# Meng-333/SRADSGAN

Measured on AMD Instinct MI355X. Metric: training images/sec (216x216, x4), higher is better.
Workload: dtype f32 (split-bf16 products: 3 bf16 MFMA terms per fp32 multiply, fp32 accumulate)

## Files before the change

### sradsgan_amd/csrc/conv_api.hip

```cpp
#include "conv_internal.h"
#include "conv_dev.h"

using namespace srhip;

namespace srhip {
struct PackEntry {
  const float* w;
  float* packed;
  int cout, cin, kh, kw, mode, fast;
};
__global__ __launch_bounds__(256) void pack_batched_kernel(const PackEntry* __restrict__ tab) {
  const PackEntry e = tab[blockIdx.y];
  const int khkw = e.kh * e.kw;
  if (e.fast) {
    constexpr int LDS_F = 32 * (16 * 9 + 1);
    __shared__ float tile[LDS_F];
    const long total = (long)e.cout * e.cin * khkw;
    const int RO = e.mode == 0 ? 8 : 32;
    const int CI = e.mode == 0 ? (khkw <= 9 ? 64 : 16) : (khkw <= 9 ? 16 : 4);
    const int ld = CI * khkw + 1;
    const int nci = (e.cin + CI - 1) / CI, nco = (e.cout + RO - 1) / RO;
    const int ndst = e.mode == 0 ? e.cout : e.cin, csrc = e.mode == 0 ? e.cin : e.cout;
    const long ndst16 = ((long)ndst + 15) / 16 * 16;
    float* s0 = e.packed;
    char* s1 = reinterpret_cast<char*>(e.packed + total);
    char* s2 = reinterpret_cast<char*>(e.packed + 2 * total);
    char* s3 = reinterpret_cast<char*>(e.packed + 3 * total);
    for (int t = blockIdx.x; t < nci * nco; t += gridDim.x) {
      const int co0 = (t / nci) * RO, ci0 = (t % nci) * CI;
      const int cw = min(CI, e.cin - ci0), rw = min(RO, e.cout - co0);
      const int rowlen = cw * khkw;
      __syncthreads();
      for (int i = threadIdx.x; i < rw * rowlen; i += 256) {
        const int r = i / rowlen, k = i - r * rowlen;
        tile[r * ld + k] = e.w[((size_t)(co0 + r) * e.cin + ci0) * khkw + k];
      }
      __syncthreads();
      auto at = [&](int a, int b, int tap) { return tile[a * ld + b * khkw + tap]; };
      const int nn = e.mode == 0 ? rw : cw, nc = e.mode == 0 ? cw : rw;
      const int n0 = e.mode == 0 ? co0 : ci0, c00 = e.mode == 0 ? ci0 : co0;
      for (int it = threadIdx.x; it < nn * khkw * (nc / 8); it += 256) {
        const int g8 = it % (nc / 8), rt = it / (nc / 8);
        const int tap = rt % khkw, dn = rt / khkw;
        float v[8];
#pragma unroll
        for (int j = 0; j < 8; ++j) v[j] = e.mode == 0 ? at(dn, g8 * 8 + j, tap) : at(g8 * 8 + j, dn, tap);
        const long idx = ((long)(n0 + dn) * khkw + tap) * csrc + c00 + g8 * 8;
        reinterpret_cast<float4*>(s0 + idx)[0] = make_float4(v[0], v[1], v[2], v[3]);
        reinterpret_cast<float4*>(s0 + idx)[1] = make_float4(v[4], v[5], v[6], v[7]);
        bf16x8_t hi, lo;
        split_bf16x8(make_float4(v[0], v[1], v[2], v[3]), make_float4(v[4], v[5], v[6], v[7]), hi, lo);
        *reinterpret_cast<u32x4*>(s1 + idx * 4) = __builtin_bit_cast(u32x4, hi);
        *reinterpret_cast<u32x4*>(s1 + idx * 4 + 16) = __builtin_bit_cast(u32x4, lo);
        const f16x8_t f16 = {(_Float16)v[0], (_Float16)v[1], (_Float16)v[2], (_Float16)v[3], (_Float16)v[4], (_Float16)v[5], (_Float16)v[6], (_Float16)v[7]};
        const u32x4 z = {0u, 0u, 0u, 0u};
        *reinterpret_cast<u32x4*>(s2 + idx * 4) = __builtin_bit_cast(u32x4, f16);
        *reinterpret_cast<u32x4*>(s2 + idx * 4 + 16) = z;
      }
      for (int it = threadIdx.x; it < nn * khkw * (nc / 16); it += 256) {
        const int dn = it % nn, rt = it / nn;
        const int tap = rt % khkw, g16 = rt / khkw;
        const int n = n0 + dn, swz = (n >> 2) & 3;
        char* row = s3 + (((long)((c00 >> 4) + g16) * khkw + tap) * ndst16 + n) * 64;
#pragma unroll
        for (int h = 0; h < 2; ++h) {
          float v[8];
#pragma unroll
          for (int j = 0; j < 8; ++j) v[j] = e.mode == 0 ? at(dn, g16 * 16 + h * 8 + j, tap) : at(g16 * 16 + h * 8 + j, dn, tap);
          bf16x8_t hi, lo;
          split_bf16x8(make_float4(v[0], v[1], v[2], v[3]), make_float4(v[4], v[5], v[6], v[7]), hi, lo);
          *reinterpret_cast<u32x4*>(row + (((2 * h) ^ swz) << 4)) = __builtin_bit_cast(u32x4, hi);
          *reinterpret_cast<u32x4*>(row + (((2 * h + 1) ^ swz) << 4)) = __builtin_bit_cast(u32x4, lo);
        }
      }
    }
  } else {
    const int csrc = e.mode == 0 ? e.cin : e.cout, cdst = e.mode == 0 ? e.cout : e.cin;
    const int ld = ((cdst + 31) / 32) * 32;
    const long total = (long)khkw * csrc * ld;
    for (long idx = (long)blockIdx.x * blockDim.x + threadIdx.x; idx < total; idx += (long)gridDim.x * blockDim.x) {
      const int row = (int)(idx / ld), col = (int)(idx - (long)row * ld);
      float v = 0.f;
      if (col < cdst) {
        const int tap = row / csrc, cs = row - tap * csrc;
        const int a = tap / e.kw, b = tap - a * e.kw;
        if (e.mode == 0)
          v = e.w[(((size_t)col * e.cin + cs) * e.kh + a) * e.kw + b];
        else
          v = e.w[(((size_t)cs * e.cin + col) * e.kh + (e.kh - 1 - a)) * e.kw + (e.kw - 1 - b)];
      }
      e.packed[idx] = v;
    }
  }
}
}

namespace srhip {
extern int g_fast_cfg;
extern int g_wgrad_cfg;
extern int g_rowtap_addr;
extern int g_rowtap_pipe;
extern int g_patch_ks;
extern int g_fast_dynlds;
extern int g_fast_ablate;
extern int g_conv_math;
extern int g_sgam_cfg;
extern int g_pers_grid;
extern int g_pers_small;
extern int g_pool_epi_any;
extern int g_pers_abl;
extern int g_phase_batch;
extern int g_headconv_rows;
}
extern int g_tail_dbg;
namespace srhip {
}

namespace srhip {
struct Probe {
  int kind = 0, n = 0, h = 0, w = 0, cin = 0, cout = 0, cap = 0, count = 0;
  hipEvent_t ev[2 * 1024];
  int units[1024];
  int created = 0;
};
static Probe g_probe;
static inline bool probe_hit(int kind, int n, int h, int w, int cin, int cout) {
  return g_probe.kind == kind && g_probe.count < g_probe.cap && g_probe.n == n && g_probe.h == h && g_probe.w == w && g_probe.cin == cin &&
         g_probe.cout == cout;
}
static inline int probe_begin(void* stream) {
  const int i = g_probe.count;
  (void)hipEventRecord(g_probe.ev[2 * i], as_stream(stream));
  return i;
}
static inline void probe_end(int i, void* stream, int units = 1) {
  (void)hipEventRecord(g_probe.ev[2 * i + 1], as_stream(stream));
  g_probe.units[i] = units;
  g_probe.count = i + 1;
}
}

extern "C" {

int srhip_probe_config(int kind, int n, int h, int w, int cin, int cout, int max_pairs) {
  SRHIP_REQUIRE(kind >= 0 && kind <= 3 && max_pairs >= 0 && max_pairs <= 1024, "probe_config: kind 0..3, max_pairs <= 1024");
  while (g_probe.created < 2 * max_pairs) {
    if (hipEventCreate(&g_probe.ev[g_probe.created]) != hipSuccess) {
      set_error("probe_config: hipEventCreate failed");
      return SRHIP_ERR_LAUNCH;
    }
    ++g_probe.created;
  }
  g_probe.kind = kind; g_probe.n = n; g_probe.h = h; g_probe.w = w; g_probe.cin = cin; g_probe.cout = cout;
  g_probe.cap = kind ? max_pairs : 0;
  g_probe.count = 0;
  return SRHIP_OK;
}
int srhip_probe_read(float* ms, int* units, int cap) {
  SRHIP_REQUIRE(ms || cap == 0, "probe_read: null buffer");
  const int n = g_probe.count < cap ? g_probe.count : cap;
  for (int i = 0; i < n; ++i) {
    if (hipEventSynchronize(g_probe.ev[2 * i + 1]) != hipSuccess || hipEventElapsedTime(&ms[i], g_probe.ev[2 * i], g_probe.ev[2 * i + 1]) != hipSuccess) {
      set_error("probe_read: event %d not readable", i);
      return -1;
    }
    if (units) units[i] = g_probe.units[i];
  }
  return n;
}

int srhip_debug_set(int key, int value) {
  if (key == 0) {
    g_fast_cfg = value;
    return SRHIP_OK;
  }
  if (key == 1) {
    g_wgrad_cfg = value;
    return SRHIP_OK;
  }
  if (key == 2) {
    g_fast_dynlds = value;
    return SRHIP_OK;
  }
  if (key == 3) {
    g_fast_ablate = value;
    return SRHIP_OK;
  }
  if (key == 4) {
    g_sgam_cfg = value;
    return SRHIP_OK;
  }
  if (key == 5) {
    g_pers_grid = value;
    return SRHIP_OK;
  }
  if (key == 6) {
    g_pers_abl = value;
    return SRHIP_OK;
  }
  if (key == 7) {
    g_tail_dbg = value;
    return SRHIP_OK;
  }
  if (key == 8) {
    g_rowtap_addr = value;
    return SRHIP_OK;
  }
  if (key == 9) {
    g_rowtap_pipe = value;
    return SRHIP_OK;
  }
  if (key == 10) {
    g_patch_ks = value;
    return SRHIP_OK;
  }
  if (key == 11) {
    g_pers_small = value;
    return SRHIP_OK;
  }
  if (key == 12) {
    g_flat_blocks = value > 0 ? value : 768;
    return SRHIP_OK;
  }
  if (key == 13) {
    g_flat_abl = value;
    return SRHIP_OK;
  }
  if (key == 14) {
    g_flat_f32_k8 = value;
    return SRHIP_OK;
  }
  if (key == 15) {
    g_patch8 = value;
    return SRHIP_OK;
  }
  if (key == 16) {
    g_patch8_abl = value;
    return SRHIP_OK;
  }
  if (key == 17) {
    g_phase_batch = value;
    return SRHIP_OK;
  }
  if (key == 18) {
    g_headconv_rows = value;
    return SRHIP_OK;
  }
  if (key == 19) {
    g_pool_epi_any = value;
    return SRHIP_OK;
  }
  return SRHIP_ERR_ARG;
}

int srhip_set_conv_math(int mode) {
  SRHIP_REQUIRE(mode == SRHIP_MATH_FP32 || mode == SRHIP_MATH_BF16X3 || mode == SRHIP_MATH_HALF, "set_conv_math: unknown mode");
  g_conv_math = mode;
  return SRHIP_OK;
}
int srhip_get_conv_math(void) { return g_conv_math; }

size_t srhip_packed_elems(int cout, int cin, int kh, int kw, int mode) {
  if (cout <= 0 || cin <= 0 || kh <= 0 || kw <= 0 || (mode != 0 && mode != 1)) return 0;
  const bool fast = mode == 0 ? fast_fwd_ok(cin, cout, kh, kw) : fast_dgrad_ok(cin, cout, kh, kw);
  if (fast)
    return 3 * (size_t)cout * cin * kh * kw + (size_t)fast_tiled_elems(mode == 0 ? cout : cin, mode == 0 ? cin : cout, kh * kw);
  const int csrc = mode == 0 ? cin : cout, cdst = mode == 0 ? cout : cin;
  return (size_t)kh * kw * csrc * legacy_packed_ld(cdst);
}

int srhip_pack_entry_bytes(void) { return (int)sizeof(PackEntry); }

int srhip_packed_is_fast(int cout, int cin, int kh, int kw, int mode) {
  return (mode == 0 ? fast_fwd_ok(cin, cout, kh, kw) : fast_dgrad_ok(cin, cout, kh, kw)) ? 1 : 0;
}

int srhip_pack_weights_batched(const void* entries_dev, int count, void* stream) {
  SRHIP_REQUIRE(entries_dev && count >= 0, "pack_weights_batched: bad argument");
  if (count == 0) return SRHIP_OK;
  hipLaunchKernelGGL(pack_batched_kernel, dim3(32, count), dim3(256), 0, as_stream(stream),
                     static_cast<const PackEntry*>(entries_dev));
  return check_launch("pack_weights_batched");
}

int srhip_pack_weight(const float* w, float* packed, int cout, int cin, int kh, int kw, int mode, void* stream) {
  SRHIP_REQUIRE(w && packed && cout > 0 && cin > 0 && kh > 0 && kw > 0 && (mode == 0 || mode == 1),
                "pack_weight: bad argument");
  const bool fast = mode == 0 ? fast_fwd_ok(cin, cout, kh, kw) : fast_dgrad_ok(cin, cout, kh, kw);
  if (fast) return fast_pack_weight(w, packed, cout, cin, kh, kw, mode, as_stream(stream));
  return legacy_pack_weight(w, packed, cout, cin, kh, kw, mode, stream);
}

int srhip_conv2d_fwd(const float* x, const float* packed, const float* bias, const float* residual,
                     const float* rowscale, const float* chanscale, float* y, int n, int h, int w, int cin, int cout, int kh, int kw,
                     int stride, int pad, int ldx, int ldy, int ldr, float slope, int flags, void* stream) {
  SRHIP_REQUIRE(x && packed && y, "conv2d_fwd: null tensor");
  SRHIP_REQUIRE(n >= 0 && h > 0 && w > 0 && cin > 0 && cout > 0 && kh > 0 && kw > 0 && stride > 0 && pad >= 0,
                "conv2d_fwd: bad geometry");
  SRHIP_REQUIRE(ldx >= cin && ldy >= cout, "conv2d_fwd: row stride smaller than channel count");
  SRHIP_REQUIRE(!(flags & SRHIP_EPI_BIAS) || bias, "conv2d_fwd: EPI_BIAS without bias");
  SRHIP_REQUIRE(!(flags & SRHIP_EPI_RESIDUAL) || (residual && ldr >= cout), "conv2d_fwd: EPI_RESIDUAL without residual");
  SRHIP_REQUIRE(!(flags & SRHIP_EPI_ROWSCALE) || rowscale, "conv2d_fwd: EPI_ROWSCALE without rowscale");
  SRHIP_REQUIRE(!(flags & SRHIP_EPI_CHANSCALE) || chanscale, "conv2d_fwd: EPI_CHANSCALE without chanscale");
  if (fast_fwd_ok(cin, cout, kh, kw)) {
    const bool pr = probe_hit(1, n, h, w, cin, cout);
    const int pi = pr ? probe_begin(stream) : 0;
    const int rc = fast_conv2d_fwd(x, packed, bias, residual, rowscale, chanscale, y, n, h, w, cin, cout, kh, kw, stride, pad, ldx, ldy,
                                   ldr, slope, flags, as_stream(stream));
    if (pr) probe_end(pi, stream);
    return rc;
  }
  SRHIP_REQUIRE(!(flags & SRHIP_EPI_CHANSCALE), "conv2d_fwd: EPI_CHANSCALE needs Cin % 16 == 0");
  return legacy_conv2d_fwd(x, packed, bias, residual, rowscale, y, n, h, w, cin, cout, kh, kw, stride, pad, ldx, ldy,
                           ldr, slope, flags, stream);
}

int srhip_conv2d_fwd_dual(const float* x, const float* packed, const float* bias, const float* residual, const float* rowscale,
                          const float* chanscale, float* y, void* y_pp, int* served, int n, int h, int w, int cin, int cout, int kh,
                          int kw, int stride, int pad, int ldx, int ldy, int ldr, float slope, int flags, void* stream) {
  SRHIP_REQUIRE(y_pp && served && (((uintptr_t)y_pp) & 15) == 0 && ldy == cout, "conv2d_fwd_dual: 16-byte aligned plane buffer, dense fp32 output");
  g_dst2_req.pp = y_pp;
  g_dst2_req.served = 0;
  const int rc = srhip_conv2d_fwd(x, packed, bias, residual, rowscale, chanscale, y, n, h, w, cin, cout, kh, kw, stride, pad, ldx, ldy, ldr,
                                  slope, flags, stream);
  *served = g_dst2_req.served;
  g_dst2_req.pp = nullptr;
  g_dst2_req.served = 0;
  return rc;
}

int srhip_conv2d_fwd_pool(const float* x, const float* packed, const float* bias, float* y, float* pool, size_t pool_sec_bytes,
                          int* nseg_out, int n, int h, int w, int cin, int cout, int ldx, int ldy, int flags, void* stream) {
  SRHIP_REQUIRE(x && packed && y && pool && nseg_out, "conv2d_fwd_pool: null tensor");
  SRHIP_REQUIRE(cout == 64 && ldy == 64 && n > 0 && h > 0 && w > 0 && cin > 0 && ldx >= cin, "conv2d_fwd_pool: 64 dense destination channels");
  SRHIP_REQUIRE((flags & ~SRHIP_EPI_BIAS) == 0 && (!(flags & SRHIP_EPI_BIAS) || bias), "conv2d_fwd_pool: plain or bias epilogue");
  SRHIP_REQUIRE(pool_sec_bytes % 16 == 0 && pool_sec_bytes < (1u << 30) && (((uintptr_t)pool) & 15) == 0 &&
                    pool_sec_bytes >= (size_t)n * POOL_MAXSEG * 64 * sizeof(float),
                "conv2d_fwd_pool: three 16-byte aligned sections of n * max_segments * 64 floats");
  g_pool_req.out = pool;
  g_pool_req.sec_bytes = (unsigned)pool_sec_bytes;
  g_pool_req.served_nseg = 0;
  const int rc = srhip_conv2d_fwd(x, packed, bias, nullptr, nullptr, nullptr, y, n, h, w, cin, cout, 3, 3, 1, 1, ldx, ldy, 0, 0.f, flags, stream);
  const int served = g_pool_req.served_nseg;
  g_pool_req.out = nullptr;
  g_pool_req.served_nseg = 0;
  if (rc != SRHIP_OK) return rc;
  if (served > 0) {
    *nseg_out = served;
    return SRHIP_OK;
  }
  *nseg_out = srhip_clam_pool_segments();
  return srhip_clam_pool_partial(y, pool, pool_sec_bytes, n, h, w, cout, stream);
}

int srhip_conv2d_dgrad(const float* dy, const float* packed, float* dx, const float* residual, const float* actmask,
                       float slope, int n, int h, int w, int cin, int cout, int kh, int kw, int stride, int pad,
                       int ldy, int ldx, int ldr, int accumulate, void* stream) {
  SRHIP_REQUIRE(dy && packed && dx, "conv2d_dgrad: null tensor");
  SRHIP_REQUIRE(n >= 0 && h > 0 && w > 0 && cin > 0 && cout > 0 && kh > 0 && kw > 0 && stride > 0 && pad >= 0,
                "conv2d_dgrad: bad geometry");
  SRHIP_REQUIRE(pad <= kh - 1 && pad <= kw - 1, "conv2d_dgrad: pad > kernel-1 unsupported");
  SRHIP_REQUIRE(ldy >= cout && ldx >= cin, "conv2d_dgrad: row stride smaller than channel count");
  SRHIP_REQUIRE(!residual || ldr >= cin, "conv2d_dgrad: residual row stride smaller than channel count");
  if (fast_dgrad_ok(cin, cout, kh, kw)) {
    const bool pr = probe_hit(2, n, h, w, cin, cout);
    const int pi = pr ? probe_begin(stream) : 0;
    const int rc = fast_conv2d_dgrad(dy, packed, dx, residual, actmask, slope, n, h, w, cin, cout, kh, kw, stride, pad, ldy,
                                     ldx, ldr, accumulate, as_stream(stream));
    if (pr) probe_end(pi, stream);
    return rc;
  }
  SRHIP_REQUIRE(!residual && !actmask, "conv2d_dgrad: fused residual/activation mask needs Cout % 16 == 0");
  return legacy_conv2d_dgrad(dy, packed, dx, n, h, w, cin, cout, kh, kw, stride, pad, ldy, ldx, accumulate, stream);
}

static int add_unserved_residuals(float* dx, const float* r2, const float* r3, long count, void* stream) {
  const float* tab[3] = {dx, r2 ? r2 : r3, r3};
  const int k = 1 + (r2 ? 1 : 0) + (r3 ? 1 : 0);
  if (k == 1) return SRHIP_OK;
  return srhip_sum_n(tab, k, dx, count, stream);
}
int srhip_conv2d_dgrad_res3(const float* dy, const float* packed, float* dx, const float* residual, const float* residual2,
                            const float* residual3, int n, int h, int w, int cin, int cout, int kh, int kw, int stride, int pad,
                            void* stream) {
  SRHIP_REQUIRE(residual && (residual2 || residual3), "conv2d_dgrad_res3: residual and at least one more");
  SRHIP_REQUIRE(cin % 4 == 0 && ((((uintptr_t)residual2) | ((uintptr_t)residual3) | ((uintptr_t)dx)) & 15) == 0, "conv2d_dgrad_res3: Cin % 4 == 0, 16-byte aligned tensors");
  g_res_req.r2 = residual2 ? residual2 : residual3;
  g_res_req.r3 = residual2 ? residual3 : nullptr;
  g_res_req.served = 0;
  const int rc = srhip_conv2d_dgrad(dy, packed, dx, residual, nullptr, 0.f, n, h, w, cin, cout, kh, kw, stride, pad, cout, cin, cin, 0, stream);
  const bool served = g_res_req.served != 0;
  g_res_req = ResRequest();
  if (rc != SRHIP_OK || served) return rc;
  return add_unserved_residuals(dx, residual2, residual3, (long)n * h * w * cin, stream);
}
int srhip_conv2d_dgrad_pp_res3(const void* dy, int dy_pp, const float* packed, float* dx, const float* residual, const float* residual2,
                               const float* residual3, int n, int h, int w, int cin, int cout, void* stream) {
  SRHIP_REQUIRE(residual && (residual2 || residual3), "conv2d_dgrad_pp_res3: residual and at least one more");
  SRHIP_REQUIRE(cin % 4 == 0 && ((((uintptr_t)residual2) | ((uintptr_t)residual3)) & 15) == 0, "conv2d_dgrad_pp_res3: Cin % 4 == 0, 16-byte aligned tensors");
  g_res_req.r2 = residual2 ? residual2 : residual3;
  g_res_req.r3 = residual2 ? residual3 : nullptr;
  g_res_req.served = 0;
// ... 209 lines not shown
```

### sradsgan_amd/csrc/conv_fast.hip

```cpp
#include "conv_dev.h"

namespace srhip {

int g_fast_ablate = 0;



template <int BM, int BN, int WM, int WN, int BK, int MATH = 0>
__global__ __launch_bounds__(WM* WN * 64) void fast_conv_kernel(const float* __restrict__ src,
                                                                 const float* __restrict__ wt,
                                                                 const float* __restrict__ bias,
                                                                 const float* __restrict__ residual,
                                                                 const float* __restrict__ rowscale,
                                                                 const float* __restrict__ chanscale,
                                                                 const float* __restrict__ actmask,
                                                                 float* __restrict__ dst, FastGeom g, int nblk_m,
                                                                 int nblk_n) {
  constexpr int NT = WM * WN * 64;
  constexpr int WTM = BM / WM, WTN = BN / WN;
  constexpr int TM = WTM / 32, TN = WTN / 32;
  constexpr int LS = BK + 4;
  constexpr int QPR = BK / 4;
  constexpr int RPP = NT / QPR;
  constexpr int AR = (BM + RPP - 1) / RPP, BR = (BN + RPP - 1) / RPP;
// ... 443 lines not shown
#pragma unroll
  for (int t = 0; t < TM; ++t) {
    const int m = m0 + wm * WTM + t * 32 + l31;
    csrow[t] = chanscale + (size_t)((m < g.M ? m : 0) / OHOW) * g.C + khalf * 4;
  }
  const int T_taps = g.TH * g.TW;
  int c_tap = 0, c_cc = 0;

  auto chunk_sync = [&](int kc) {
    if (kc + 1 < nk)
      asm volatile("s_waitcnt vmcnt(%0)" ::"n"(AI + BI) : "memory");
    else
      asm volatile("s_waitcnt vmcnt(0)" ::: "memory");
    __builtin_amdgcn_s_barrier();
    asm volatile("" ::: "memory");
  };
  auto read_frags = [&](int stage, float4 (&af)[2][TM], float4 (&bf)[2][TN]) {
    const char* sb = lds + stage * STAGE_B;
#pragma unroll
    for (int t = 0; t < TM; ++t) af[0][t] = *reinterpret_cast<const float4*>(sb + aoff[t]);
#pragma unroll
    for (int u = 0; u < TN; ++u) bf[0][u] = *reinterpret_cast<const float4*>(sb + boff[u]);
#pragma unroll
    for (int t = 0; t < TM; ++t) af[1][t] = *reinterpret_cast<const float4*>(sb + (aoff[t] ^ (MATH ? 16 : 32)));
#pragma unroll
    for (int u = 0; u < TN; ++u) bf[1][u] = *reinterpret_cast<const float4*>(sb + (boff[u] ^ (MATH ? 16 : 32)));
    if (cscale) {
#pragma unroll
      for (int ks = 0; ks < 2; ++ks)
#pragma unroll
        for (int t = 0; t < TM; ++t) {
          const float4 sc = *reinterpret_cast<const float4*>(csrow[t] + c_cc * BK + (MATH ? ks * 4 + khalf * 4 : ks * 8));
          af[ks][t].x *= sc.x;
          af[ks][t].y *= sc.y;
          af[ks][t].z *= sc.z;
          af[ks][t].w *= sc.w;
        }
      if (++c_tap == T_taps) {
        c_tap = 0;
        ++c_cc;
      }
    }
  };

  if (MATH == 0 && nk > 0) {
    issue(0);
    if (nk > 1) issue(1);
    int stage = 0, nstage = 2;
    for (int kc = 0; kc < nk; ++kc) {
      chunk_sync(kc);
      if (kc + 2 < nk) issue(nstage);
      float4 af[2][TM], bf[2][TN];
      read_frags(stage, af, bf);
#pragma unroll
      for (int ks = 0; ks < 2; ++ks) {
#pragma unroll
        for (int t = 0; t < TM; ++t)
#pragma unroll
          for (int u = 0; u < TN; ++u) acc[t][u] = mfma32f(af[ks][t].x, bf[ks][u].x, acc[t][u]);
#pragma unroll
        for (int t = 0; t < TM; ++t)
#pragma unroll
          for (int u = 0; u < TN; ++u) acc[t][u] = mfma32f(af[ks][t].y, bf[ks][u].y, acc[t][u]);
#pragma unroll
        for (int t = 0; t < TM; ++t)
#pragma unroll
          for (int u = 0; u < TN; ++u) acc[t][u] = mfma32f(af[ks][t].z, bf[ks][u].z, acc[t][u]);
#pragma unroll
        for (int t = 0; t < TM; ++t)
#pragma unroll
          for (int u = 0; u < TN; ++u) acc[t][u] = mfma32f(af[ks][t].w, bf[ks][u].w, acc[t][u]);
      }
      stage = stage == 2 ? 0 : stage + 1;
      nstage = nstage == 2 ? 0 : nstage + 1;
    }
  }
  if (MATH >= 1 && nk > 0) {
    constexpr int PROD = MATH >= 1 ? MATH - 1 : 0;
    issue(0);
    if (nk > 1) issue(1);
    int stage = 0, nstage = 2;
    for (int kc = 0; kc < nk; ++kc) {
      chunk_sync(kc);
      if (kc + 2 < nk) issue(nstage);
      float4 af[2][TM], bf[2][TN];
      read_frags(stage, af, bf);
      bf16x8_t ah[TM], al[TM], bh[TN], bl[TN];
#pragma unroll
      for (int t = 0; t < TM; ++t) {
        if (PROD == 0) split_bf16x8(af[0][t], af[1][t], ah[t], al[t]);
        else ah[t] = al[t] = round16x8<PROD>(af[0][t], af[1][t]);
      }
#pragma unroll
      for (int u = 0; u < TN; ++u) {
        bh[u] = __builtin_bit_cast(bf16x8_t, bf[0][u]);
        bl[u] = PROD == 0 ? __builtin_bit_cast(bf16x8_t, bf[1][u]) : bh[u];
      }
#pragma unroll
      for (int i = 0; i < nprod<PROD>() * TM * TN; ++i) {
        const int grp = PROD == 0 ? i / (TM * TN) : 2, t = (i % (TM * TN)) / TN, u = i % TN;
        acc[t][u] = mma16<PROD>(grp == 0 ? al[t] : ah[t], grp == 1 ? bl[u] : bh[u], acc[t][u]);
      }
      stage = stage == 2 ? 0 : stage + 1;
      nstage = nstage == 2 ? 0 : nstage + 1;
    }
  }

  const int flags = EPI >= 0 ? EPI : g.flags;
  __syncthreads();
  float* wl = reinterpret_cast<float*>(lds) + wave * (32 * WTN);
  constexpr int QPRW = WTN / 4;
  constexpr int NRD = 32 * QPRW / 64;
#pragma unroll
  for (int t = 0; t < TM; ++t) {
#pragma unroll
    for (int u = 0; u < TN; ++u)
#pragma unroll
      for (int r = 0; r < 16; ++r) wl[((r & 3) + 8 * (r >> 2) + 4 * khalf) * WTN + u * 32 + l31] = acc[t][u][r];
    asm volatile("s_waitcnt lgkmcnt(0)" ::: "memory");
    constexpr int EB = NRD < 4 ? NRD : 4;
#pragma unroll
    for (int i0 = 0; i0 < NRD; i0 += EB) {
      float4 vq[EB];
      EpiOps eo[EB];
      unsigned dpx[EB];
      int nq[EB];
      bool okq[EB];
#pragma unroll
      for (int j = 0; j < EB; ++j) {
        const int idx = (i0 + j) * 64 + lane;
        const int row = idx / QPRW, cq = idx - row * QPRW;
        vq[j] = *reinterpret_cast<const float4*>(wl + row * WTN + cq * 4);
        const int m = m0 + wm * WTM + t * 32 + row;
        nq[j] = n0 + wn * WTN + cq * 4;
        okq[j] = m < g.M && nq[j] < g.K;
        size_t dpix = (size_t)(okq[j] ? m : 0);
        if (!g.dst_identity) {
          const int mm = okq[j] ? m : 0;
          const int nimg = mm / OHOW;
          const int rem = mm - nimg * OHOW;
          const int oh = rem / g.OW;
          const int ow = rem - oh * g.OW;
          dpix = ((size_t)nimg * g.Hd + (oh * g.dsd + g.ph)) * g.Wd + (ow * g.dsd + g.pw);
        }
        dpx[j] = (unsigned)dpix;
        if (!okq[j]) nq[j] = 0;
        eo[j] = epi_fetch(dpix, nq[j], flags, g, bias, residual, rowscale, actmask, dst, EPI < 0 && g.accumulate != 0);
      }
#pragma unroll
      for (int j = 0; j < EB; ++j)
        if (okq[j]) epi_finish(vq[j], eo[j], dpx[j], nq[j], flags, g, dst, EPI < 0 && g.accumulate != 0);
    }
    if (t + 1 < TM) asm volatile("s_waitcnt lgkmcnt(0)" ::: "memory");
  }
}


template <int BN, int EPI, int PROD = 0>
__global__ __launch_bounds__(256) __attribute__((amdgpu_waves_per_eu(3))) void conv_patch_kernel(const float* __restrict__ src, const float* __restrict__ wt,
                                                          const float* __restrict__ bias,
                                                          const float* __restrict__ residual,
                                                          const float* __restrict__ actmask, float* __restrict__ dst,
                                                          FastGeom g, PatchGeom pg, int nblk_m, int nblk_n) {
  constexpr int NW = 4, BK = 16;
  constexpr int WTM = 64, WTN = BN / 2;
  constexpr int TM = WTM / 32, TN = WTN / 32;
  constexpr int BPW = BN / 64;
  constexpr int MAXP = 3;
  constexpr int PATCH_B = 12 * 1024;
  constexpr int BSTAGE_B = BN * 64;
  constexpr int EPI_B = NW * 32 * WTN * 4;
  constexpr int LDS_B = 2 * PATCH_B + 3 * BSTAGE_B > EPI_B ? 2 * PATCH_B + 3 * BSTAGE_B : EPI_B;
  __shared__ __attribute__((aligned(1024))) char lds[LDS_B];
  __shared__ int pix_tab[128];

  const int tid = threadIdx.x, lane = tid & 63;
  const int wave = __builtin_amdgcn_readfirstlane(tid >> 6);
  const int tile = xcd_tile(blockIdx.x, nblk_m * nblk_n);
  const int tile_n = tile % nblk_n, pid = tile / nblk_n;
  const int n0 = tile_n * BN;
  const int tpi = pg.tiles_h * pg.tiles_w;
  const int img = pid / tpi;
  const int prem = pid - img * tpi;
  const int ty = prem / pg.tiles_w, tx = prem - ty * pg.tiles_w;
  const int oh0 = ty * pg.PH, ow0 = tx * pg.PW;
  const unsigned lds_base = (unsigned)(size_t)(__attribute__((address_space(3))) char*)lds;
  if (tid < 128) {
    int pr_, pc_;
    patch_pixel(tid, pg.PH, pg.PW, pg.gmap, pr_, pc_);
    pix_tab[tid] = (pr_ << 16) | pc_;
  }
  __syncthreads();

  const int swz = (lane >> 4) & 3;
  const int aq = (lane & 3) ^ swz;
  int abase[MAXP];
#pragma unroll
  for (int k = 0; k < MAXP; ++k) {
    const int row = (k * NW + wave) * 16 + (lane >> 2);
    abase[k] = -1;
    if (row < pg.PR) {
      const int pi = row / pg.PWP, pj = row - pi * pg.PWP;
      const int sh = oh0 + pg.lo_h + pi, sw = ow0 + pg.lo_w + pj;
      if (sh >= 0 && sh < g.Hs && sw >= 0 && sw < g.Ws) abase[k] = ((img * g.Hs + sh) * g.Ws + sw) * g.lds + aq * 4;
    }
  }
  int bbase[BPW];
  bool bval[BPW];
#pragma unroll
  for (int j = 0; j < BPW; ++j) {
    const int n = n0 + wave * 16 * BPW + 16 * j + (lane >> 2);
    bval[j] = n < g.K;
    bbase[j] = n * g.ldw + aq * 4;
  }
  const unsigned a_dst = __builtin_amdgcn_readfirstlane(lds_base + wave * 1024);
  const unsigned b_dst = __builtin_amdgcn_readfirstlane(lds_base + 2 * PATCH_B + wave * BPW * 1024);

  const int CC = g.C / BK;
  int wtap[9];
#pragma unroll
  for (int t = 0; t < 9; ++t) wtap[t] = ((g.kh0 + (t / 3) * g.khs) * g.KW + (g.kw0 + (t % 3) * g.kws)) * g.C;

  __amdgpu_buffer_rsrc_t rs_a = __builtin_amdgcn_make_buffer_rsrc(const_cast<float*>(src), 0, g.src_bytes, 0x00020000);
  __amdgpu_buffer_rsrc_t rs_b = __builtin_amdgcn_make_buffer_rsrc(const_cast<float*>(wt), 0, g.w_bytes, 0x00020000);
  unsigned aoffb[MAXP], boffb[BPW];
#pragma unroll
  for (int k = 0; k < MAXP; ++k) aoffb[k] = abase[k] >= 0 ? (unsigned)abase[k] * 4u : F_OOB;
#pragma unroll
  for (int j = 0; j < BPW; ++j) boffb[j] = bval[j] ? (unsigned)bbase[j] * 4u : F_OOB;
  auto issue_a = [&](int buf, int k, int cc) {
    lds_dma16_buf(aoffb[k] + (unsigned)(cc * BK * 4), rs_a, a_dst + buf * PATCH_B + k * (NW * 1024));
  };
  auto issue_b = [&](int stage, int tap, int cc) {
    const int wk = wtap[tap] + cc * BK;
#pragma unroll
    for (int j = 0; j < BPW; ++j) lds_dma16_buf(boffb[j] + (unsigned)(wk * 4), rs_b, b_dst + stage * BSTAGE_B + j * 1024);
  };
  auto convert_piece = [&](int buf, int k) {
    float4* slot = reinterpret_cast<float4*>(lds + buf * PATCH_B + (k * NW + wave) * 1024 + lane * 16);
    const float4 own = *slot;
    float4 oth;
    oth.x = __builtin_bit_cast(float, __builtin_amdgcn_mov_dpp(__builtin_bit_cast(int, own.x), 0xB1, 0xF, 0xF, true));
    oth.y = __builtin_bit_cast(float, __builtin_amdgcn_mov_dpp(__builtin_bit_cast(int, own.y), 0xB1, 0xF, 0xF, true));
    oth.z = __builtin_bit_cast(float, __builtin_amdgcn_mov_dpp(__builtin_bit_cast(int, own.z), 0xB1, 0xF, 0xF, true));
    oth.w = __builtin_bit_cast(float, __builtin_amdgcn_mov_dpp(__builtin_bit_cast(int, own.w), 0xB1, 0xF, 0xF, true));
    const bool odd = aq & 1;
    bf16x8_t hi, lo;
    if (PROD == 0) {
      split_bf16x8(odd ? oth : own, odd ? own : oth, hi, lo);
      *reinterpret_cast<bf16x8_t*>(slot) = odd ? lo : hi;
    } else if (!odd) {
      *reinterpret_cast<bf16x8_t*>(slot) = round16x8<PROD>(own, oth);
    }
  };

#pragma unroll
  for (int k = 0; k < MAXP; ++k) issue_a(0, k, 0);
  issue_b(0, 0, 0);
  issue_b(1, 1, 0);

  const int wm = wave >> 1, wn = wave & 1;
  const int khalf = lane >> 5, l31 = lane & 31;
  int aoff[9][TM];
#pragma unroll
  for (int t = 0; t < TM; ++t) {
    const int r = wm * WTM + t * 32 + l31;
    const int pt = pix_tab[r];
    const int orow = pt >> 16, ocol = pt & 0xffff;
    const int arow = orow < pg.PH ? orow * pg.PWP + ocol : 0;
#pragma unroll
    for (int tap = 0; tap < 9; ++tap) {
      const int a_th = (g.dh0 + (tap / 3) * g.dhs) - pg.lo_h, a_tw = (g.dw0 + (tap % 3) * g.dws) - pg.lo_w;
      const int pr = arow + a_th * pg.PWP + a_tw;
      aoff[tap][t] = pr * 64 + (((2 * khalf) ^ ((pr >> 2) & 3)) << 4);
    }
  }
  int boff[TN];
#pragma unroll
  for (int u = 0; u < TN; ++u) {
    const int row = wn * WTN + u * 32 + l31;
    boff[u] = 2 * PATCH_B + row * 64 + (((2 * khalf) ^ ((row >> 2) & 3)) << 4);
  }
  f32x16 acc[TM][TN];
#pragma unroll
  for (int t = 0; t < TM; ++t)
#pragma unroll
    for (int u = 0; u < TN; ++u)
#pragma unroll
      for (int r = 0; r < 16; ++r) acc[t][u][r] = 0.f;

  auto do_tap = [&](auto tapc, auto lastc, int cc) {
    constexpr int TAP = decltype(tapc)::value;
    constexpr bool LAST = decltype(lastc)::value != 0;
    constexpr int NEWER = ((LAST && TAP == 8) ? 0 : BPW) + ((!LAST && TAP >= 1 && TAP <= MAXP) ? 1 : 0);
    wait_vmcnt<NEWER>();
    asm volatile("s_waitcnt lgkmcnt(0)" ::: "memory");
    __builtin_amdgcn_s_barrier();
    asm volatile("" ::: "memory");
    const int pbuf = cc & 1;
    if (!LAST && TAP < MAXP) issue_a(pbuf ^ 1, TAP, cc + 1);
    if (TAP + 2 < 9) issue_b((TAP + 2) % 3, TAP + 2, cc);
    else if (!LAST) issue_b((TAP + 2) % 3, TAP + 2 - 9, cc + 1);
    if (!LAST && TAP >= 2 && TAP - 2 < MAXP) convert_piece(pbuf ^ 1, TAP - 2);
    const char* pb = lds + pbuf * PATCH_B;
    const char* sb = lds + (TAP % 3) * BSTAGE_B;
    bf16x8_t ah[TM], al[TM], bh[TN], bl[TN];
// ... 1457 lines not shown
  }
}

static bool shape_ok(int csrc, int kh, int kw) { return csrc % 16 == 0 && kh * kw <= 32 && kh == kw; }
bool fast_fwd_ok(int cin, int cout, int kh, int kw) { return shape_ok(cin, kh, kw); }
bool fast_dgrad_ok(int cin, int cout, int kh, int kw) { return shape_ok(cout, kh, kw); }
bool fast_wgrad_ok(int cin, int cout, int kh, int kw) { return cin % 16 == 0 && cout % 4 == 0 && kh == kw; }

int fast_pack_weight(const float* w, float* packed, int cout, int cin, int kh, int kw, int mode, hipStream_t st) {
  const long total = (long)cout * cin * kh * kw;
  hipLaunchKernelGGL(fast_pack_kernel, dim3(cdiv(total, 256)), dim3(256), 0, st, w, packed, cout, cin, kh, kw, mode);
  return check_launch("fast_pack_weight");
}

thread_local Dst2Request g_dst2_req;
thread_local ResRequest g_res_req;
thread_local PhaseRequest g_phase_req;
int g_conv_math = 0;
int g_fast_dynlds = 0;
template <int BM, int BN, int WM, int WN, int BK>
static int launch_fast(const float* src, const float* wt, const float* bias, const float* residual,
                       const float* rowscale, const float* chanscale, const float* actmask, float* dst,
                       const FastGeom& g, hipStream_t st) {
  const int nbm = cdiv(g.M, BM), nbn = cdiv(g.K, BN);
  hipLaunchKernelGGL((fast_conv_kernel<BM, BN, WM, WN, BK>), dim3(nbm * nbn), dim3(WM * WN * 64), g_fast_dynlds, st, src, wt, bias,
                     residual, rowscale, chanscale, actmask, dst, g, nbm, nbn);
  return check_launch("fast_conv");
}

__global__ __launch_bounds__(256) void dot_conv_kernel(const float* __restrict__ src, const float* __restrict__ wt,
                                                        const float* __restrict__ bias, float* __restrict__ dst, FastGeom g) {
  const int lane = threadIdx.x & 63;
  const int m = blockIdx.x * 4 + (threadIdx.x >> 6);
  if (m >= g.M) return;
  const int ow = m % g.OW, t = m / g.OW;
  const int oh = t % g.OH, n = t / g.OH;
  float acc = 0.f;
  for (int th = 0; th < g.TH; ++th) {
    const int sh = oh * g.ss + g.dh0 + th * g.dhs;
    if (sh < 0 || sh >= g.Hs) continue;
    for (int tw = 0; tw < g.TW; ++tw) {
      const int sw = ow * g.ss + g.dw0 + tw * g.dws;
      if (sw < 0 || sw >= g.Ws) continue;
      const float* xp = src + ((size_t)(n * g.Hs + sh) * g.Ws + sw) * g.lds;
      const float* wp = wt + (size_t)((g.kh0 + th * g.khs) * g.KW + (g.kw0 + tw * g.kws)) * g.C;
      for (int c = lane * 4; c < g.C; c += 256) {
        const float4 a = *reinterpret_cast<const float4*>(xp + c);
        const float4 b = *reinterpret_cast<const float4*>(wp + c);
        acc = fmaf(a.x, b.x, acc);
        acc = fmaf(a.y, b.y, acc);
        acc = fmaf(a.z, b.z, acc);
        acc = fmaf(a.w, b.w, acc);
      }
    }
  }
#pragma unroll
  for (int o = 32; o >= 1; o >>= 1) acc += __shfl_xor(acc, o, 64);
  if (lane == 0) {
    float v = acc;
    if (g.flags & SRHIP_EPI_BIAS) v += bias[0];
    if (g.flags & SRHIP_EPI_LRELU) v = v > 0.f ? v : v * g.slope;
    dst[((size_t)(n * g.Hd + oh * g.dsd + g.ph) * g.Wd + ow * g.dsd + g.pw) * g.ldd] = v;
  }
}

int g_patch_ks = 1;
int g_fast_cfg = 0;
int g_phase_batch = 1;

static bool plan_patch(const FastGeom& g, PatchGeom* pg, double min_eff = 0.70) {
  if (g.TH != 3 || g.TW != 3 || g.ss != 1 || g.dsd != 1 || g.ph != 0 || g.pw != 0) return false;
  if ((g.dhs != 1 && g.dhs != -1) || (g.dws != 1 && g.dws != -1)) return false;
  if (g.Hd != g.OH || g.Wd != g.OW) return false;
  double best = 0.0;
  for (int pw = 4; pw <= 64 && pw <= g.OW + 3; ++pw) {
    int ph = 128 / pw;
    if (ph > g.OH) ph = g.OH;
    if (ph < 1 || (ph + 2) * (pw + 2) > 192) continue;
    const long tiles = (long)cdiv(g.OH, ph) * cdiv(g.OW, pw);
    const double eff = (double)g.OH * g.OW / ((double)tiles * 128.0) + 1e-6 * (double)(pw - pw % 16) / pw;
    if (eff > best + 1e-9) {
      best = eff;
      pg->PH = ph; pg->PW = pw;
    }
  }
  if (best < min_eff || best <= 0.0) return false;
  pg->tiles_h = cdiv(g.OH, pg->PH);
  pg->tiles_w = cdiv(g.OW, pg->PW);
  pg->PWP = pg->PW + 2;
  pg->PR = (pg->PH + 2) * pg->PWP;
  pg->npieces = cdiv(pg->PR, 16);
  pg->lo_h = g.dhs > 0 ? g.dh0 : g.dh0 + 2 * g.dhs;
  pg->lo_w = g.dws > 0 ? g.dw0 : g.dw0 + 2 * g.dws;
  const int a = pg->PW >> 4;
  const int nfull = pg->PH * a < 8 ? pg->PH * a : 8;
  auto base = [&](int q) { return ((q / a) * pg->PWP + (q % a) * 16) & 15; };
  int fin[8], nf = 0, singles[8], ns = 0;
  bool used[8] = {false, false, false, false, false, false, false, false};
  for (int q = 0; q < nfull; ++q) {
    if (used[q]) continue;
    used[q] = true;
    int partner = -1;
    for (int p2 = q + 1; p2 < nfull; ++p2)
      if (!used[p2] && base(p2) == base(q)) {
        partner = p2;
        break;
      }
    if (partner >= 0) {
      used[partner] = true;
      fin[nf++] = q;
      fin[nf++] = partner;
    } else {
      singles[ns++] = q;
    }
  }
  for (int i = 0; i < ns; ++i) fin[nf++] = singles[i];
  for (int q = nfull; q < 8; ++q) fin[nf++] = q;
  pg->gmap = 0;
  for (int i = 0; i < 8; ++i) pg->gmap |= (unsigned)(fin[i] & 15) << (4 * i);
  return true;
}

long pp_sign_tiles(int n, int h, int w, int cout) {
  if (cout < 128 || cout % 128 != 0) return 0;
  FastGeom g;
  g.TH = 3; g.TW = 3; g.ss = 1; g.dsd = 1; g.ph = 0; g.pw = 0; g.dhs = 1; g.dws = 1; g.dh0 = -1; g.dw0 = -1;
  g.Hd = g.OH = h; g.Wd = g.OW = w;
  PatchGeom pg;
  if (!plan_patch(g, &pg, 0.0)) return 0;
  return (long)n * pg.tiles_h * pg.tiles_w * (cout / 128);
}

static int run_fast(const float* src, const float* wt, const float* bias, const float* residual,
                    const float* rowscale, const float* chanscale, const float* actmask, float* dst, const FastGeom& g,
                    hipStream_t st) {
  if (g.M <= 0) return SRHIP_OK;
  if (g.src_pp || g.dst_pp) {
    PatchGeom pg;
    const int ef = g.flags & 0x3f;
    if (g_conv_math == 1 && g.K >= 64 && g.K % 8 == 0 && g.C % 32 == 0 && !(ef & (SRHIP_EPI_CHANSCALE | SRHIP_EPI_ROWSCALE)) && !g.accumulate &&
        plan_patch(g, &pg, 0.0)) {
      const int nbm = g.N * pg.tiles_h * pg.tiles_w;
      const bool wide = g.K >= 128;
      const int nbn = cdiv(g.K, wide ? 128 : 64);
      if (wide && !residual) {
        const int rc8 = launch_patch8(src, wt, bias, actmask, dst, g, pg, nbm, ef, st);
        if (rc8 >= 0) return rc8;
      }
      const int rc = launch_patch_pers(src, wt, bias, residual, actmask, dst, g, pg, nbm, nbn, wide, 0, ef, st);
      if (rc >= 0) return rc;
    }
    set_error("conv2d (padded planes): shape / arithmetic mode not served by the persistent patch kernel");
    return SRHIP_ERR_ARG;
  }
#define SRHIP_LF(BM_, BN_, WM_, WN_, BK_) \
  return launch_fast<BM_, BN_, WM_, WN_, BK_>(src, wt, bias, residual, rowscale, chanscale, actmask, dst, g, st)
  if (g.K <= 4 && g_fast_cfg != 20 && g_fast_cfg != 22 && g.TH == 3 && g.TW == 3 && g.ss == 1 && g.dsd == 1 && g.ph == 0 &&
      g.pw == 0 && g.Hd == g.OH && g.Wd == g.OW && (g.dhs == 1 || g.dhs == -1) && (g.dws == 1 || g.dws == -1) &&
      !(g.flags & ~(SRHIP_EPI_BIAS | SRHIP_EPI_LRELU | SRHIP_EPI_GRADDATA)) && !g.accumulate && g.M >= 65536) {
    const int th = cdiv(g.OH, 16), tw = cdiv(g.OW, 16);
    const int lo_h = g.dhs > 0 ? g.dh0 : g.dh0 + 2 * g.dhs, lo_w = g.dws > 0 ? g.dw0 : g.dw0 + 2 * g.dws;
    if (g.K == 3)
      hipLaunchKernelGGL((narrow_conv_kernel<3>), dim3(g.N * th * tw), dim3(256), 0, st, src, wt, bias, dst, g, th, tw, lo_h, lo_w);
    else
      hipLaunchKernelGGL((narrow_conv_kernel<4>), dim3(g.N * th * tw), dim3(256), 0, st, src, wt, bias, dst, g, th, tw, lo_h, lo_w);
    return check_launch("narrow_conv");
  }
  if (g.K == 1 && g.C % 4 == 0 && g.lds % 4 == 0 && (((uintptr_t)src | (uintptr_t)wt) & 15) == 0 && g.M < 65536 && g_fast_cfg != 20 &&
      g_fast_cfg != 22 && !(g.flags & ~(SRHIP_EPI_BIAS | SRHIP_EPI_LRELU | SRHIP_EPI_GRADDATA)) && !g.accumulate) {
    hipLaunchKernelGGL(dot_conv_kernel, dim3(cdiv(g.M, 4)), dim3(256), 0, st, src, wt, bias, dst, g);
    return check_launch("dot_conv");
  }
  const int prod = g_conv_math == 2 ? ((g.flags & SRHIP_EPI_GRADDATA) ? 1 : 2) : 0;
  const float* w16 = wt + (size_t)(g.w_bytes >> 2) * (prod == 2 ? 2 : 1);
  if (g.K <= 32 && g_conv_math >= 1 && g_fast_cfg != 20 && !(g.flags & (SRHIP_EPI_CHANSCALE | 0x300))) {
    const int nbm = cdiv(g.M, 128), nbn = cdiv(g.K, 32);
    if (prod == 0)
      hipLaunchKernelGGL((fast_conv_kernel<128, 32, 4, 1, 16, 1>), dim3(nbm * nbn), dim3(256), g_fast_dynlds, st, src,
                         w16, bias, residual, rowscale, chanscale, actmask, dst, g, nbm, nbn);
    else if (prod == 1)
      hipLaunchKernelGGL((fast_conv_kernel<128, 32, 4, 1, 16, 2>), dim3(nbm * nbn), dim3(256), g_fast_dynlds, st, src,
                         w16, bias, residual, rowscale, chanscale, actmask, dst, g, nbm, nbn);
    else
      hipLaunchKernelGGL((fast_conv_kernel<128, 32, 4, 1, 16, 3>), dim3(nbm * nbn), dim3(256), g_fast_dynlds, st, src,
                         w16, bias, residual, rowscale, chanscale, actmask, dst, g, nbm, nbn);
    return check_launch("fast_conv");
  }
  if (g.K <= 32) SRHIP_LF(128, 32, 4, 1, 16);
  const int eflags = g.flags & 0x3f;
  const bool al16 = g.K % 4 == 0 && g.ldd % 4 == 0 && ((uintptr_t)dst & 15) == 0 && (!residual || (g.ldr % 4 == 0 && ((uintptr_t)residual & 15) == 0)) &&
                    (!actmask || ((uintptr_t)actmask & 15) == 0) && (!bias || ((uintptr_t)bias & 15) == 0);
  bool patch_to_dma = false;
  if (g_conv_math >= 1 && g_fast_cfg != 20 && g_fast_cfg != 21 && (g_fast_cfg < 1 || g_fast_cfg == 23 || g_fast_cfg == 24) && !(g.flags & 0x300) && g.K >= 64 && al16 &&
      !(eflags & (SRHIP_EPI_CHANSCALE | SRHIP_EPI_ROWSCALE)) && !g.accumulate) {
    PatchGeom pg;
    if (plan_patch(g, &pg)) {
      const int nbm = g.N * pg.tiles_h * pg.tiles_w;
      const bool wide = g.K >= 128 && g_fast_cfg != 24;
      const int nbn = cdiv(g.K, wide ? 128 : 64);
      if (g_fast_cfg == 23) {
        patch_to_dma = (long)nbm * nbn >= 256;
      } else if ((long)nbm * nbn >= 256 || g_fast_cfg == -2) {
        const float* wsplit = w16;
        if (!(g.flags & 0x400) && wide && prod == 0 && !residual && g_fast_cfg != 23) {
          const int rc8 = launch_patch8(src, wt, bias, actmask, dst, g, pg, nbm, eflags, st);
          if (rc8 >= 0) return rc8;
        }
        if (!(g.flags & 0x400)) {
          const int rc = launch_patch_pers(src, wt, bias, residual, actmask, dst, g, pg, nbm, nbn, wide, prod, eflags, st);
          if (rc >= 0) return rc;
        }
        if (prod != 0) {
#define SRHIP_LPH(BN_, PROD_)                                                                                       \
  do {                                                                                                              \
    hipLaunchKernelGGL((conv_patch_kernel<BN_, -1, PROD_>), dim3(nbm * nbn), dim3(256), 0, st, src, wsplit, bias,   \
                       residual, actmask, dst, g, pg, nbm, nbn);                                                   \
    return check_launch("conv_patch");                                                                              \
  } while (0)
          if (wide && prod == 1) SRHIP_LPH(128, 1);
          if (wide) SRHIP_LPH(128, 2);
          if (prod == 1) SRHIP_LPH(64, 1);
          SRHIP_LPH(64, 2);
#undef SRHIP_LPH
        }
#define SRHIP_LP(BN_, EPI_)                                                                                         \
  do {                                                                                                              \
    hipLaunchKernelGGL((conv_patch_kernel<BN_, EPI_>), dim3(nbm * nbn), dim3(256), 0, st, src, wsplit, bias,       \
                       residual, actmask, dst, g, pg, nbm, nbn);                                                   \
    return check_launch("conv_patch");                                                                              \
  } while (0)
#define SRHIP_LPE(BN_)                                                  \
  do {                                                                  \
    if (eflags == 0) SRHIP_LP(BN_, 0);                                  \
    if (eflags == SRHIP_EPI_BIAS) SRHIP_LP(BN_, 1);                     \
    if (eflags == (SRHIP_EPI_BIAS | SRHIP_EPI_LRELU)) SRHIP_LP(BN_, 3); \
    if (eflags == SRHIP_EPI_ACTMASK) SRHIP_LP(BN_, 32);                 \
    if (eflags == SRHIP_EPI_RESIDUAL) SRHIP_LP(BN_, 4);                 \
    SRHIP_LP(BN_, -1);                                                  \
  } while (0)
        if (wide) SRHIP_LPE(128);
        if (g_patch_ks && g.C % 32 == 0 && g.C >= 32) {
#define SRHIP_LK(EPI_)                                                                                              \
  do {                                                                                                              \
    hipLaunchKernelGGL((conv_patch_ks_kernel<EPI_>), dim3(nbm * nbn), dim3(256), 0, st, src, wsplit, bias, residual, \
                       actmask, dst, g, pg, nbm, nbn);                                                             \
    return check_launch("conv_patch_ks");                                                                           \
  } while (0)
          if (eflags == 0) SRHIP_LK(0);
          if (eflags == SRHIP_EPI_BIAS) SRHIP_LK(1);
          if (eflags == SRHIP_EPI_RESIDUAL) SRHIP_LK(4);
          SRHIP_LK(-1);
#undef SRHIP_LK
        }
        SRHIP_LPE(64);
#undef SRHIP_LPE
#undef SRHIP_LP
      }
    }
  }
  if (g_fast_cfg != 20 && (g_fast_cfg < 1 || g_fast_cfg == 23 || g_fast_cfg == 24) && !(g.flags & 0x300) && g.K >= 64 && al16 &&
      (!(eflags & SRHIP_EPI_CHANSCALE) || ((uintptr_t)chanscale & 15) == 0)) {
    const int nbm = cdiv(g.M, 128);
    const bool force = g_fast_cfg == -1 || patch_to_dma;
    const long min_tiles = g_conv_math >= 1 ? 128 : 512;
    const bool wide = g.K >= 128 && ((long)nbm * cdiv(g.K, 128) >= min_tiles || force);
    const long b64 = (long)nbm * cdiv(g.K, 64);
    if (wide || b64 >= min_tiles || force) {
#define SRHIP_LD(BN_, EPI_)                                                                                        \
  do {                                                                                                             \
    const int nbn = cdiv(g.K, BN_);                                                                                \
    if (g.dst2_pp) g_dst2_req.served = 1;                                                                          \
    PhaseSet ps_;                                                                                                  \
    int grid_ = nbm * nbn;                                                                                         \
    if (g_phase_req.active) {                            \
      ps_ = g_phase_req.ps;                                                                                        \
      grid_ = 0;                                                                                                   \
      for (int k_ = 0; k_ < ps_.n; ++k_) {                                                                         \
        ps_.first[k_] = grid_;                                                                                     \
        grid_ += ps_.p[k_].nblk_m * nbn;                                                                           \
      }                                                                                                            \
      ps_.first[ps_.n] = grid_;                                                                                    \
      g_phase_req.launched = 1;                                                                                    \
    }                                                                                                              \
    if (g_conv_math == 1) {                                                                                        \
      hipLaunchKernelGGL((fast_conv_dma_kernel<128, BN_, EPI_, 1>), dim3(grid_), dim3(256), g_fast_dynlds, st,     \
                         src, w16, bias, residual, rowscale, chanscale, actmask, dst, g, nbm,                      \
                         nbn, ps_);                                                                                \
    } else                                                                                                         \
      hipLaunchKernelGGL((fast_conv_dma_kernel<128, BN_, EPI_, 0>), dim3(grid_), dim3(256), g_fast_dynlds, st,     \
                         src, wt, bias, residual, rowscale, chanscale, actmask, dst, g, nbm, nbn, ps_);            \
    return check_launch("fast_conv_dma");                                                                          \
  } while (0)
#define SRHIP_LDE(BN_)                                                  \
  do {                                                                  \
    if (g.accumulate) SRHIP_LD(BN_, -1);                                \
    if (eflags == 0) SRHIP_LD(BN_, 0);                                  \
    if (eflags == SRHIP_EPI_BIAS) SRHIP_LD(BN_, 1);                     \
    if (eflags == (SRHIP_EPI_BIAS | SRHIP_EPI_LRELU)) SRHIP_LD(BN_, 3); \
    if (eflags == SRHIP_EPI_ACTMASK) SRHIP_LD(BN_, 32);                 \
    if (eflags == SRHIP_EPI_RESIDUAL) SRHIP_LD(BN_, 4);                 \
    if (eflags == 29) SRHIP_LD(BN_, 29);  \
    SRHIP_LD(BN_, -1);                                                  \
  } while (0)
      if (prod != 0) {
#define SRHIP_LDH(BN_, MATH_)                                                                                       \
  do {                                                                                                              \
// ... 482 lines not shown
```

Measured before the change: 665.8.

## Add specialized 1x1 conv kernel for 64-to-64 channel layers

Adds a dedicated kernel for 1x1 convolutions with 64 input and 64 output channels. It keeps the whole split-bf16 weight fragment set resident in LDS, has each wave stream 32-pixel tiles with register prefetch of the next tile, and does the bf16x3 MFMA products and a staged epilogue. It is enabled by default when the problem is large, replacing the generic fast GEMM tiling for these layers. Risks are lower occupancy from the LDS footprint and correctness gaps in edge epilogue paths such as chanscale with many images.

After: 666.4 (median of 6 runs). Within noise of the previous version (+0.1%).

```diff
diff --git a/sradsgan_amd/csrc/conv_api.hip b/sradsgan_amd/csrc/conv_api.hip
--- a/sradsgan_amd/csrc/conv_api.hip
+++ b/sradsgan_amd/csrc/conv_api.hip
@@ -111,6 +111,7 @@
 extern int g_pers_abl;
 extern int g_phase_batch;
 extern int g_headconv_rows;
+extern int g_c64;
 }
 extern int g_tail_dbg;
 namespace srhip {
@@ -248,6 +249,10 @@
   }
   if (key == 19) {
     g_pool_epi_any = value;
+    return SRHIP_OK;
+  }
+  if (key == 20) {
+    g_c64 = value;
     return SRHIP_OK;
   }
   return SRHIP_ERR_ARG;
diff --git a/sradsgan_amd/csrc/conv_fast.hip b/sradsgan_amd/csrc/conv_fast.hip
--- a/sradsgan_amd/csrc/conv_fast.hip
+++ b/sradsgan_amd/csrc/conv_fast.hip
@@ -619,6 +619,114 @@
         if (okq[j]) epi_finish(vq[j], eo[j], dpx[j], nq[j], flags, g, dst, EPI < 0 && g.accumulate != 0);
     }
     if (t + 1 < TM) asm volatile("s_waitcnt lgkmcnt(0)" ::: "memory");
+  }
+}
+
+int g_c64 = 1;
+constexpr int C64_RS = 72;
+constexpr int C64_STG = 8 * C64_RS;
+constexpr int C64_FRAG = 16 * 64 * 4;
+constexpr int C64_MAX_N = 32;
+
+template <int EPI>
+__global__ __launch_bounds__(256) void conv1x1_c64_kernel(const float* __restrict__ src, const float* __restrict__ w16,
+                                                          const float* __restrict__ bias, const float* __restrict__ residual,
+                                                          const float* __restrict__ rowscale, const float* __restrict__ chanscale,
+                                                          const float* __restrict__ actmask, float* __restrict__ dst, FastGeom g,
+                                                          int ntiles) {
+  extern __shared__ __attribute__((aligned(16))) float c64_lds[];
+  const int lane = threadIdx.x & 63, h = lane >> 5, l31 = lane & 31;
+  const int wave = __builtin_amdgcn_readfirstlane(threadIdx.x >> 6);
+  const int flags = EPI >= 0 ? EPI : g.flags;
+  const bool cscale = (flags & SRHIP_EPI_CHANSCALE) != 0;
+  const bool accum = EPI < 0 && g.accumulate != 0;
+  float* frag = c64_lds;
+  float* stg = c64_lds + C64_FRAG + wave * C64_STG;
+  float* cs = c64_lds + C64_FRAG + 4 * C64_STG;
+#pragma unroll
+  for (int i = 0; i < 4; ++i) {
+    const int k = wave + 4 * i, u = k >> 3, cc = (k >> 1) & 3, lo = k & 1;
+    reinterpret_cast<float4*>(frag)[k * 64 + lane] =
+        *reinterpret_cast<const float4*>(w16 + (size_t)(32 * u + l31) * g.ldw + cc * 16 + 8 * h + 4 * lo);
+  }
+  if (cscale)
+    for (int i = threadIdx.x; i < g.N * 16; i += 256) reinterpret_cast<float4*>(cs)[i] = reinterpret_cast<const float4*>(chanscale)[i];
+  __syncthreads();
+  auto bfrag = [&](int u, int cc, int lo) {
+    return __builtin_bit_cast(bf16x8_t, reinterpret_cast<const float4*>(frag)[((u * 4 + cc) * 2 + lo) * 64 + lane]);
+  };
+
+  __amdgpu_buffer_rsrc_t rs = __builtin_amdgcn_make_buffer_rsrc(const_cast<float*>(src), 0, g.src_bytes, 0x00020000);
+  auto aoff = [&](int tile, int cc, int s) -> unsigned {
+    const int p = tile * 32 + l31;
+    return (tile < ntiles && p < g.M) ? ((unsigned)p * (unsigned)g.lds + (unsigned)(cc * 16 + 8 * h + 4 * s)) * 4u : F_OOB;
+  };
+  const int tstride = gridDim.x * 4;
+  int tile = blockIdx.x * 4 + wave;
+  float4 a[4][2];
+#pragma unroll
+  for (int cc = 0; cc < 4; ++cc)
+#pragma unroll
+    for (int s = 0; s < 2; ++s) a[cc][s] = bufload4(rs, aoff(tile, cc, s));
+  const int OHOW = g.OH * g.OW;
+
+  for (; tile < ntiles; tile += tstride) {
+    const int next = tile + tstride;
+    const int p = tile * 32 + l31;
+    const float* csrow = cs + ((p < g.M ? p : 0) / OHOW) * 64 + 8 * h;
+    f32x16 acc0, acc1;
+#pragma unroll
+    for (int r = 0; r < 16; ++r) acc0[r] = acc1[r] = 0.f;
+#pragma unroll
+    for (int cc = 0; cc < 4; ++cc) {
+      float4 x0 = a[cc][0], x1 = a[cc][1];
+      if (cscale) {
+        const float4 s0 = *reinterpret_cast<const float4*>(csrow + cc * 16), s1 = *reinterpret_cast<const float4*>(csrow + cc * 16 + 4);
+        x0.x *= s0.x; x0.y *= s0.y; x0.z *= s0.z; x0.w *= s0.w;
+        x1.x *= s1.x; x1.y *= s1.y; x1.z *= s1.z; x1.w *= s1.w;
+      }
+      bf16x8_t ah, al;
+      split_bf16x8(x0, x1, ah, al);
+      a[cc][0] = bufload4(rs, aoff(next, cc, 0));
+      a[cc][1] = bufload4(rs, aoff(next, cc, 1));
+      const bf16x8_t bh0 = bfrag(0, cc, 0), bh1 = bfrag(1, cc, 0), bl0 = bfrag(0, cc, 1), bl1 = bfrag(1, cc, 1);
+      acc0 = mma16<0>(al, bh0, acc0);
+      acc1 = mma16<0>(al, bh1, acc1);
+      acc0 = mma16<0>(ah, bl0, acc0);
+      acc1 = mma16<0>(ah, bl1, acc1);
+      acc0 = mma16<0>(ah, bh0, acc0);
+      acc1 = mma16<0>(ah, bh1, acc1);
+    }
+
+#pragma unroll
+    for (int q = 0; q < 4; ++q) {
+#pragma unroll
+      for (int j = 0; j < 4; ++j) {
+        stg[(4 * h + j) * C64_RS + l31] = acc0[4 * q + j];
+        stg[(4 * h + j) * C64_RS + 32 + l31] = acc1[4 * q + j];
+      }
+      asm volatile("s_waitcnt lgkmcnt(0)" ::: "memory");
+      float4 vq[2];
+      EpiOps eo[2];
+      unsigned dpx[2];
+      int nq[2];
+      bool okq[2];
+#pragma unroll
+      for (int i = 0; i < 2; ++i) {
+        const int idx = i * 64 + lane;
+        const int row = idx >> 4, cq = idx & 15;
+        vq[i] = *reinterpret_cast<const float4*>(stg + row * C64_RS + cq * 4);
+        const int m = tile * 32 + 8 * q + row;
+        okq[i] = m < g.M;
+        dpx[i] = (unsigned)(okq[i] ? m : 0);
+        nq[i] = cq * 4;
+        eo[i] = epi_fetch(dpx[i], nq[i], flags, g, bias, residual, rowscale, actmask, dst, accum);
+      }
+#pragma unroll
+      for (int i = 0; i < 2; ++i)
+        if (okq[i]) epi_finish(vq[i], eo[i], dpx[i], nq[i], flags, g, dst, accum);
+      asm volatile("s_waitcnt lgkmcnt(0)" ::: "memory");
+    }
   }
 }
 
@@ -2382,6 +2490,29 @@
     }
     set_error("conv2d (padded planes): shape / arithmetic mode not served by the persistent patch kernel");
     return SRHIP_ERR_ARG;
+  }
+  if (g_c64 && g_conv_math == 1 && ((g_fast_cfg == 0 && cdiv(g.M, 128) >= 128) || g_fast_cfg == -1) && g.TH == 1 && g.TW == 1 && g.ss == 1 && g.dsd == 1 && g.dst_identity &&
+      g.dh0 == 0 && g.dw0 == 0 && g.kh0 == 0 && g.kw0 == 0 && g.C == 64 && g.K == 64 && g.ldw == 64 && g.lds % 4 == 0 && g.ldd % 4 == 0 &&
+      !(g.flags & 0x300) && !g_phase_req.active && ((uintptr_t)dst & 15) == 0 && (!residual || (g.ldr % 4 == 0 && ((uintptr_t)residual & 15) == 0)) &&
+      (!actmask || ((uintptr_t)actmask & 15) == 0) && (!bias || ((uintptr_t)bias & 15) == 0) &&
+      (!(g.flags & SRHIP_EPI_CHANSCALE) || (g.N <= C64_MAX_N && ((uintptr_t)chanscale & 15) == 0))) {
+    const float* w16 = wt + (size_t)(g.w_bytes >> 2);
+    const int ntiles = cdiv(g.M, 32);
+    int blocks = cdiv(ntiles, 4);
+    if (g_c64 > 1 && blocks > g_c64) blocks = g_c64;
+    const int ef = g.flags & 0x3f;
+    const size_t lds = (size_t)(C64_FRAG + 4 * C64_STG) * 4 + ((ef & SRHIP_EPI_CHANSCALE) ? (size_t)g.N * 64 * 4 : 0);
+    if (g.dst2_pp) g_dst2_req.served = 1;
+    if (!g.accumulate && ef == 0)
+      hipLaunchKernelGGL((conv1x1_c64_kernel<0>), dim3(blocks), dim3(256), lds, st, src, w16, bias, residual, rowscale, chanscale,
+                         actmask, dst, g, ntiles);
+    else if (!g.accumulate && ef == 29)
+      hipLaunchKernelGGL((conv1x1_c64_kernel<29>), dim3(blocks), dim3(256), lds, st, src, w16, bias, residual, rowscale, chanscale,
+                         actmask, dst, g, ntiles);
+    else
+      hipLaunchKernelGGL((conv1x1_c64_kernel<-1>), dim3(blocks), dim3(256), lds, st, src, w16, bias, residual, rowscale, chanscale,
+                         actmask, dst, g, ntiles);
+    return check_launch("conv1x1_c64");
   }
 #define SRHIP_LF(BM_, BN_, WM_, WN_, BK_) \
   return launch_fast<BM_, BN_, WM_, WN_, BK_>(src, wt, bias, residual, rowscale, chanscale, actmask, dst, g, st)
```
